# Y-Claw/Multilevel-GNN

Hardware: AMD Instinct MI355X
Metric: graphs/sec fwd+bwd, 3-level GNN on 10k-node d=128 synthetic; HBM GB/s %peak (higher is better)
Workload: dtype f32; 1 GPU; configs[1]: ER graphs N=10000 E=160000 x64 per GPU, d=128, 3 GENConv(softmax, res+, LayerNorm) + projection pooling G=25000 k=2 + DiffPool 146->37->10, fp32; step = CSR build (of the next batch, on a second stream) + fwd + bwd + grad all-reduce + Adam; graphs_per_gpu=64, global_batch=64, parallelism=dp1, world_size=1, allreduce_bytes=1429768

## Files before the change

multilevel-gnn_amd/csrc/densesage.hip:

```cpp
#include "common.h"
#include "mlgnn.h"
#include "tile_gemm.h"

namespace mlgnn {

constexpr int kDsMaxN = 160, kDsMaxC = 128, kDsMaxO = 64, kDsMaxNAdj = 48;
constexpr int kDsBlock = 1024, kDsWaves = kDsBlock / kWave;
constexpr int kDsSO = kDsMaxO + 1;
constexpr float kDsNormEps = 1e-12f;

struct DsArgs {
  const void* x; const void* adj; const void* w_rel; const void* w_root; const float* bias;
  const void* gy; const void* y; const float* rinv_in;
  void* y_out; float* rinv; void* gx; void* gadj; float* ws;
  int n; int C; int O; int adj_batched; int normalize; int ws_cols;
};

template <typename AB>
__device__ __forceinline__ void ds_degrees(const AB ab, int n, float* deg, float* raw) {
  const int lane = threadIdx.x & (kWave - 1), wave = threadIdx.x / kWave;
  for (int r = wave; r < n; r += kDsWaves) {
    float s = 0.f;
    for (int j = lane; j < n; j += kWave) s += ab[(size_t)r * n + j];
#pragma unroll
    for (int off = 32; off > 0; off >>= 1) s += __shfl_xor(s, off);
    if (lane == 0) {
      if (raw) raw[r] = s;
      deg[r] = fmaxf(s, 1.0f);
    }
  }
}

struct DsLds { int so, sx, np; };
__host__ __device__ inline DsLds ds_lds(int n, int C, int O) {
  DsLds l;
  l.np = (n + 15) & ~15;
  l.so = ((O + 15) & ~15) + 1;
  l.sx = C + 1 + (C & 1);
  return l;
}
inline size_t ds_fwd_lds_bytes(int n, int C, int O) {
  const DsLds l = ds_lds(n, C, O);
  return ((size_t)l.np * l.so + (size_t)l.np * l.sx + l.np) * 4;
}
inline size_t ds_bwd_lds_bytes(int n, int C, int O, bool adj_grad) {
  const DsLds l = ds_lds(n, C, O);
  size_t f = (size_t)2 * l.np * l.so + 2 * l.np;
  if (adj_grad) f += (size_t)l.np * l.so + (size_t)l.np * (l.np + 1);
  return f * 4;
}

template <typename T>
__global__ __launch_bounds__(kDsBlock) void dense_sage_fwd_kernel(const DsArgs p) {
  extern __shared__ __attribute__((aligned(16))) float ds_smem[];
  const int b = blockIdx.x, tid = threadIdx.x;
  const int lane = tid & (kWave - 1), wave = tid / kWave;
  const int n = p.n, C = p.C, O = p.O;
  const DsLds L = ds_lds(n, C, O);
  const int SO = L.so, SX = L.sx;
  float* Pm_ = ds_smem;
  float* Xm_ = Pm_ + (size_t)L.np * SO;
  float* deg = Xm_ + (size_t)L.np * SX;
#define P(r, c) Pm_[(r) * SO + (c)]
#define X(r, c) Xm_[(r) * SX + (c)]
  const StoredIn<T> xb{static_cast<const T*>(p.x) + (size_t)b * n * C};
  const StoredIn<T> ab{static_cast<const T*>(p.adj) + (p.adj_batched ? (size_t)b * n * n : 0)};
  const StoredIn<T> w_rel{static_cast<const T*>(p.w_rel)}, w_root{static_cast<const T*>(p.w_root)};
  const int NP = (n + 15) & ~15, OP = (O + 15) & ~15;
  const int Nt = NP / 16, Ot = OP / 16;
  const int l15 = lane & 15, lq = lane >> 4;

  ds_degrees(ab, n, deg, nullptr);
  for (int idx = tid; idx < NP * C; idx += kDsBlock) {
    const int r = idx / C, c = idx % C;
    X(r, c) = r < n ? xb[idx] : 0.f;
  }
  __syncthreads();
  for (int t = wave; t < Nt * Ot; t += kDsWaves) {
    const int i0 = (t / Ot) * 16, j0 = (t % Ot) * 16;
    const f32x4 acc = tile_gemm(C,
        [&](int i, int k) { return k < C ? X(i0 + i, k) : 0.f; },
        [&](int k, int j) { return (j0 + j < O && k < C) ? w_rel[(size_t)(j0 + j) * C + k] : 0.f; });
#pragma unroll
    for (int r = 0; r < 4; ++r) P(i0 + lq * 4 + r, j0 + l15) = acc[r];
  }
  __syncthreads();
  f32x4 keep[(kDsMaxN / 16) * (kDsMaxO / 16) / kDsWaves + 1];
  int nk = 0;
  for (int t = wave; t < Nt * Ot; t += kDsWaves, ++nk) {
    const int i0 = (t / Ot) * 16, j0 = (t % Ot) * 16;
    f32x4 acc = tile_gemm(n,
        [&](int i, int k) { return (i0 + i < n && k < n) ? ab[(size_t)(i0 + i) * n + k] : 0.f; },
        [&](int k, int j) { return k < n ? P(k, j0 + j) : 0.f; });
    const f32x4 root = tile_gemm(C,
        [&](int i, int k) { return k < C ? X(i0 + i, k) : 0.f; },
        [&](int k, int j) { return (j0 + j < O && k < C) ? w_root[(size_t)(j0 + j) * C + k] : 0.f; });
    const float bj = (p.bias && j0 + l15 < O) ? p.bias[j0 + l15] : 0.f;
#pragma unroll
    for (int r = 0; r < 4; ++r) {
      const int row = i0 + lq * 4 + r;
      acc[r] = acc[r] / deg[min(row, n - 1)] + root[r] + bj;
    }
    keep[nk] = acc;
  }
  __syncthreads();
  nk = 0;
  for (int t = wave; t < Nt * Ot; t += kDsWaves, ++nk) {
    const int i0 = (t / Ot) * 16, j0 = (t % Ot) * 16;
#pragma unroll
    for (int r = 0; r < 4; ++r) P(i0 + lq * 4 + r, j0 + l15) = keep[nk][r];
  }
  __syncthreads();
  for (int r = wave; r < n; r += kDsWaves) {
    const float v = lane < O ? P(r, lane) : 0.f;
    float ss = v * v;
#pragma unroll
    for (int off = 32; off > 0; off >>= 1) ss += __shfl_xor(ss, off);
    const float ri = p.normalize ? 1.0f / fmaxf(sqrtf(ss), kDsNormEps) : 1.0f;
    if (lane < O) stored_write<T>(p.y_out, ((size_t)b * n + r) * O + lane, v * ri);
    if (lane == 0) p.rinv[(size_t)b * n + r] = ri;
  }
}
#undef P
#undef X

template <typename T>
__global__ __launch_bounds__(kDsBlock) void dense_sage_bwd_kernel(const DsArgs p) {
  extern __shared__ __attribute__((aligned(16))) float ds_smem[];
  const int b = blockIdx.x, tid = threadIdx.x;
  const int lane = tid & (kWave - 1), wave = tid / kWave;
  const int n = p.n, C = p.C, O = p.O;
  const DsLds L = ds_lds(n, C, O);
  const int SO = L.so, SM = L.np + 1;
  float* G_ = ds_smem;
  float* GP_ = G_ + (size_t)L.np * SO;
  float* deg = GP_ + (size_t)L.np * SO;
  float* raw = deg + L.np;
  float* Pm_ = raw + L.np;
  float* M_ = Pm_ + (size_t)L.np * SO;
#define G(r, c) G_[(r) * SO + (c)]
#define GP(r, c) GP_[(r) * SO + (c)]
#define Pm(r, c) Pm_[(r) * SO + (c)]
#define M(r, c) M_[(r) * SM + (c)]
  const StoredIn<T> xb{static_cast<const T*>(p.x) + (size_t)b * n * C};
  const StoredIn<T> ab{static_cast<const T*>(p.adj) + (p.adj_batched ? (size_t)b * n * n : 0)};
  const StoredIn<T> w_rel{static_cast<const T*>(p.w_rel)}, w_root{static_cast<const T*>(p.w_root)};
  const StoredIn<T> gyb{static_cast<const T*>(p.gy) + (size_t)b * n * O};
  const StoredIn<T> yb{static_cast<const T*>(p.y) + (size_t)b * n * O};
  const int NP = (n + 15) & ~15, OP = (O + 15) & ~15, CP = (C + 15) & ~15;
  const int Nt = NP / 16, Ot = OP / 16, Ct = CP / 16;
  const int l15 = lane & 15, lq = lane >> 4;

  ds_degrees(ab, n, deg, raw);
  for (int r = wave; r < NP; r += kDsWaves) {
    float gv = 0.f, yv = 0.f;
    if (r < n && lane < O) { gv = gyb[(size_t)r * O + lane]; yv = yb[(size_t)r * O + lane]; }
    float dot = gv * yv;
#pragma unroll
    for (int off = 32; off > 0; off >>= 1) dot += __shfl_xor(dot, off);
    const float ri = r < n ? p.rinv_in[(size_t)b * n + r] : 0.f;
    const float g = p.normalize ? (gv - yv * dot) * ri : gv;
    if (lane < OP) G(r, lane) = (r < n && lane < O) ? g : 0.f;
  }
  __syncthreads();
  for (int t = wave; t < Nt * Ot; t += kDsWaves) {
    const int i0 = (t / Ot) * 16, j0 = (t % Ot) * 16;
    const f32x4 acc = tile_gemm(n,
        [&](int i, int k) { return (i0 + i < n && k < n) ? ab[(size_t)k * n + i0 + i] : 0.f; },
        [&](int k, int j) { return k < n ? G(k, j0 + j) / deg[k] : 0.f; });
#pragma unroll
    for (int r = 0; r < 4; ++r) GP(i0 + lq * 4 + r, j0 + l15) = acc[r];
  }
  __syncthreads();
  const size_t gx_off = (size_t)b * n * C;
  for (int t = wave; t < Nt * Ct; t += kDsWaves) {
    const int i0 = (t / Ct) * 16, c0 = (t % Ct) * 16;
    f32x4 acc = tile_gemm(O,
        [&](int i, int k) { return k < O ? GP(i0 + i, k) : 0.f; },
        [&](int k, int j) { return (k < O && c0 + j < C) ? w_rel[(size_t)k * C + c0 + j] : 0.f; });
    const f32x4 t2 = tile_gemm(O,
        [&](int i, int k) { return k < O ? G(i0 + i, k) : 0.f; },
        [&](int k, int j) { return (k < O && c0 + j < C) ? w_root[(size_t)k * C + c0 + j] : 0.f; });
#pragma unroll
    for (int r = 0; r < 4; ++r) {
      const int row = i0 + lq * 4 + r, col = c0 + l15;
      if (row < n && col < C) stored_write<T>(p.gx, gx_off + (size_t)row * C + col, acc[r] + t2[r]);
    }
  }
  float* wsb = p.ws + (size_t)b * p.ws_cols;
  for (int t = wave; t < 2 * Ot * Ct; t += kDsWaves) {
    const int which = t / (Ot * Ct), tt = t % (Ot * Ct);
    const int o0 = (tt / Ct) * 16, c0 = (tt % Ct) * 16;
    const float* src = which == 0 ? GP_ : G_;
    const f32x4 acc = tile_gemm(n,
        [&](int i, int k) { return k < n ? src[k * SO + o0 + i] : 0.f; },
        [&](int k, int j) { return (k < n && c0 + j < C) ? xb[(size_t)k * C + c0 + j] : 0.f; });
#pragma unroll
    for (int r = 0; r < 4; ++r) {
      const int o = o0 + lq * 4 + r, c = c0 + l15;
      if (o < O && c < C) wsb[(size_t)which * O * C + (size_t)o * C + c] = acc[r];
    }
  }
  for (int o = tid; o < O; o += kDsBlock) {
    float s = 0.f;
    for (int r = 0; r < n; ++r) s += G(r, o);
    wsb[(size_t)2 * O * C + o] = s;
  }
  if (p.gadj) {
    for (int t = wave; t < Nt * Ot; t += kDsWaves) {
      const int i0 = (t / Ot) * 16, j0 = (t % Ot) * 16;
      const f32x4 acc = tile_gemm(C,
          [&](int i, int k) { return (i0 + i < n && k < C) ? xb[(size_t)(i0 + i) * C + k] : 0.f; },
          [&](int k, int j) { return (j0 + j < O && k < C) ? w_rel[(size_t)(j0 + j) * C + k] : 0.f; });
#pragma unroll
      for (int r = 0; r < 4; ++r) Pm(i0 + lq * 4 + r, j0 + l15) = acc[r];
    }
    __syncthreads();
    for (int t = wave; t < Nt * Nt; t += kDsWaves) {
      const int i0 = (t / Nt) * 16, j0 = (t % Nt) * 16;
      const f32x4 acc = tile_gemm(O,
          [&](int i, int k) { return k < O ? G(i0 + i, k) : 0.f; },
          [&](int k, int j) { return k < O ? Pm(j0 + j, k) : 0.f; });
#pragma unroll
      for (int r = 0; r < 4; ++r) M(i0 + lq * 4 + r, j0 + l15) = acc[r];
    }
    __syncthreads();
    const size_t ga_off = (size_t)b * n * n;
    for (int r = wave; r < n; r += kDsWaves) {
      float c = lane < n ? ab[(size_t)r * n + lane] * M(r, lane) : 0.f;
#pragma unroll
      for (int off = 32; off > 0; off >>= 1) c += __shfl_xor(c, off);
      const float ci = raw[r] > 1.0f ? c / deg[r] : 0.f;
      if (lane < n) stored_write<T>(p.gadj, ga_off + (size_t)r * n + lane, (M(r, lane) - ci) / deg[r]);
    }
  }
}
#undef G
#undef GP
#undef Pm
#undef M

static bool ds_dims_ok(int64_t n, int64_t C, int64_t O) {
  return n >= 1 && n <= kDsMaxN && C >= 1 && C <= kDsMaxC && O >= 1 && O <= kDsMaxO;
}

}

using namespace mlgnn;

extern "C" int mlgnn_dense_sage_supported(int64_t n, int64_t C, int64_t O, int need_grad_adj) {
  return (ds_dims_ok(n, C, O) && (!need_grad_adj || n <= kDsMaxNAdj)) ? 1 : 0;
}

extern "C" int64_t mlgnn_dense_sage_bwd_workspace_floats(int64_t B, int64_t C, int64_t O) {
  if (B < 0 || C <= 0 || O <= 0) return MLGNN_E_SHAPE;
  return B * (2 * O * C + O);
}

extern "C" int mlgnn_dense_sage_fwd(const void* x, const void* adj, const void* w_rel, const void* w_root,
                                    const float* bias, void* y, float* rinv, int64_t B, int64_t n, int64_t C,
                                    int64_t O, int adj_batched, int normalize, int dtype, void* stream) {
  if (dtype != MLGNN_DTYPE_F32 && dtype != MLGNN_DTYPE_BF16) return MLGNN_E_DTYPE;
  if (B < 0 || !ds_dims_ok(n, C, O)) return MLGNN_E_SHAPE;
  if (B == 0) return 0;
  if (!x || !adj || !w_rel || !w_root || !y || !rinv) return MLGNN_E_NULL;
  DsArgs a = {};
  a.x = x; a.adj = adj; a.w_rel = w_rel; a.w_root = w_root;
  a.bias = bias; a.y_out = y; a.rinv = rinv;
  a.n = (int)n; a.C = (int)C; a.O = (int)O; a.adj_batched = adj_batched; a.normalize = normalize;
  const size_t lds = ds_fwd_lds_bytes((int)n, (int)C, (int)O);
  static size_t fwd_attr = 0;
  if (lds > fwd_attr) {
    const int most = (int)ds_fwd_lds_bytes(kDsMaxN, kDsMaxC, kDsMaxO);
    (void)hipFuncSetAttribute(reinterpret_cast<const void*>(&dense_sage_fwd_kernel<float>), hipFuncAttributeMaxDynamicSharedMemorySize, most);
    (void)hipFuncSetAttribute(reinterpret_cast<const void*>(&dense_sage_fwd_kernel<bf16_t>), hipFuncAttributeMaxDynamicSharedMemorySize, most);
    fwd_attr = (size_t)most;
  }
  if (dtype == MLGNN_DTYPE_BF16) hipLaunchKernelGGL(dense_sage_fwd_kernel<bf16_t>, dim3((unsigned)B), dim3(kDsBlock), lds, (hipStream_t)stream, a);
  else hipLaunchKernelGGL(dense_sage_fwd_kernel<float>, dim3((unsigned)B), dim3(kDsBlock), lds, (hipStream_t)stream, a);
  return (int)hipGetLastError();
}

extern "C" int mlgnn_dense_sage_bwd(const void* grad_y, const void* y, const float* rinv, const void* x,
                                    const void* adj, const void* w_rel, const void* w_root, void* grad_x,
                                    void* grad_adj, float* grad_w, float* workspace, int64_t workspace_floats,
                                    int64_t B, int64_t n, int64_t C, int64_t O, int adj_batched, int normalize,
                                    int dtype, void* stream) {
  if (dtype != MLGNN_DTYPE_F32 && dtype != MLGNN_DTYPE_BF16) return MLGNN_E_DTYPE;
  if (B < 0 || !ds_dims_ok(n, C, O)) return MLGNN_E_SHAPE;
  if (grad_adj && n > kDsMaxNAdj) return MLGNN_E_SHAPE;
  if (!grad_w) return MLGNN_E_NULL;
  const int cols = (int)(2 * O * C + O);
  hipStream_t s = (hipStream_t)stream;
  if (B == 0) return (int)hipMemsetAsync(grad_w, 0, (size_t)cols * 4, s);
  if (!grad_y || !y || !rinv || !x || !adj || !w_rel || !w_root || !grad_x || !workspace) return MLGNN_E_NULL;
  if (workspace_floats < B * cols) return MLGNN_E_WORKSPACE;
  DsArgs a = {};
  a.x = x; a.adj = adj; a.w_rel = w_rel; a.w_root = w_root;
  a.gy = grad_y; a.y = y; a.rinv_in = rinv;
  a.gx = grad_x; a.gadj = grad_adj; a.ws = workspace; a.ws_cols = cols;
  a.n = (int)n; a.C = (int)C; a.O = (int)O; a.adj_batched = adj_batched; a.normalize = normalize;
  const size_t lds = ds_bwd_lds_bytes((int)n, (int)C, (int)O, grad_adj != nullptr);
  static size_t bwd_attr = 0;
  if (lds > bwd_attr) {
    const size_t most = ds_bwd_lds_bytes(kDsMaxN, kDsMaxC, kDsMaxO, false) > ds_bwd_lds_bytes(kDsMaxNAdj, kDsMaxC, kDsMaxO, true)
                            ? ds_bwd_lds_bytes(kDsMaxN, kDsMaxC, kDsMaxO, false) : ds_bwd_lds_bytes(kDsMaxNAdj, kDsMaxC, kDsMaxO, true);
    (void)hipFuncSetAttribute(reinterpret_cast<const void*>(&dense_sage_bwd_kernel<float>), hipFuncAttributeMaxDynamicSharedMemorySize, (int)most);
    (void)hipFuncSetAttribute(reinterpret_cast<const void*>(&dense_sage_bwd_kernel<bf16_t>), hipFuncAttributeMaxDynamicSharedMemorySize, (int)most);
    bwd_attr = most;
  }
  if (dtype == MLGNN_DTYPE_BF16) hipLaunchKernelGGL(dense_sage_bwd_kernel<bf16_t>, dim3((unsigned)B), dim3(kDsBlock), lds, s, a);
  else hipLaunchKernelGGL(dense_sage_bwd_kernel<float>, dim3((unsigned)B), dim3(kDsBlock), lds, s, a);
  int err = (int)hipGetLastError();
  if (err) return err;
  launch_reduce_partials(workspace, grad_w, (int)B, cols, s);
  return (int)hipGetLastError();
}
```

multilevel-gnn_amd/csrc/tile_gemm.h:

```cpp
#pragma once
#include "common.h"

namespace mlgnn {

using f32x4 = __attribute__((ext_vector_type(4))) float;

constexpr int kTileUnroll = 8;

template <typename FA, typename FB>
__device__ __forceinline__ f32x4 tile_gemm(int kdim, FA a_at, FB b_at) {
  const int lane = threadIdx.x & (kWave - 1);
  const int l15 = lane & 15, lk = lane >> 4;
  f32x4 acc = {0.f, 0.f, 0.f, 0.f};
  for (int k0 = 0; k0 < kdim; k0 += 4 * kTileUnroll) {
    float a[kTileUnroll], b[kTileUnroll];
#pragma unroll
    for (int u = 0; u < kTileUnroll; ++u) {
      a[u] = a_at(l15, k0 + 4 * u + lk);
      b[u] = b_at(k0 + 4 * u + lk, l15);
    }
#pragma unroll
    for (int u = 0; u < kTileUnroll; ++u) acc = __builtin_amdgcn_mfma_f32_16x16x4f32(a[u], b[u], acc, 0, 0, 0);
  }
  return acc;
}

}
```

Before: 5504 graphs/s.

## Stage dense SAGE operands in LDS and interleave two MFMA tiles per wave

The DiffPool dense SAGE forward and backward kernels now copy x, the adjacency and both weight matrices into LDS through a multi-row staging helper, instead of having every MFMA tile reread them from global memory. The GEMMs run through a new LDS tile_gemm that computes two independent accumulators at once, and degree sums are taken from the staged adjacency. LDS regions are reused through explicit layout plans, and the row count per wave is a template parameter with a small-n variant. This cuts redundant global loads and exposes more MFMA ILP, at the cost of more LDS and register pressure and more complex buffer aliasing.

```diff
diff --git a/multilevel-gnn_amd/csrc/densesage.hip b/multilevel-gnn_amd/csrc/densesage.hip
--- a/multilevel-gnn_amd/csrc/densesage.hip
+++ b/multilevel-gnn_amd/csrc/densesage.hip
@@ -16,128 +16,234 @@
   int n; int C; int O; int adj_batched; int normalize; int ws_cols;
 };
 
-template <typename AB>
-__device__ __forceinline__ void ds_degrees(const AB ab, int n, float* deg, float* raw) {
+constexpr int kDsRows = kDsMaxN / kDsWaves, kDsRowsSmall = 3;
+template <int ROWS>
+__device__ __forceinline__ void ds_degrees(const float* adj, int sa, int n, float* deg, float* raw, float (&sum)[ROWS]) {
   const int lane = threadIdx.x & (kWave - 1), wave = threadIdx.x / kWave;
-  for (int r = wave; r < n; r += kDsWaves) {
-    float s = 0.f;
-    for (int j = lane; j < n; j += kWave) s += ab[(size_t)r * n + j];
-#pragma unroll
-    for (int off = 32; off > 0; off >>= 1) s += __shfl_xor(s, off);
-    if (lane == 0) {
-      if (raw) raw[r] = s;
-      deg[r] = fmaxf(s, 1.0f);
-    }
-  }
-}
-
-struct DsLds { int so, sx, np; };
-__host__ __device__ inline DsLds ds_lds(int n, int C, int O) {
-  DsLds l;
-  l.np = (n + 15) & ~15;
-  l.so = ((O + 15) & ~15) + 1;
-  l.sx = C + 1 + (C & 1);
+#pragma unroll
+  for (int u = 0; u < ROWS; ++u) sum[u] = 0.f;
+  for (int j = lane; j < n; j += kWave) {
+#pragma unroll
+    for (int u = 0; u < ROWS; ++u) sum[u] += adj[min(wave + u * kDsWaves, n - 1) * sa + j];
+  }
+#pragma unroll
+  for (int off = 32; off > 0; off >>= 1) {
+#pragma unroll
+    for (int u = 0; u < ROWS; ++u) sum[u] += __shfl_xor(sum[u], off);
+  }
+#pragma unroll
+  for (int u = 0; u < ROWS; ++u) {
+    const int r = wave + u * kDsWaves;
+    if (lane == 0 && r < n) {
+      if (raw) raw[r] = sum[u];
+      deg[r] = fmaxf(sum[u], 1.0f);
+    }
+  }
+}
+template <int ROWS>
+__device__ __forceinline__ void ds_degrees(const float* adj, int sa, int n, float* deg) {
+  float sum[ROWS];
+  ds_degrees<ROWS>(adj, sa, n, deg, nullptr, sum);
+}
+
+constexpr int kDsLdsFloats = 40000;
+constexpr int kDsMaxKeep = 4;
+
+struct DsFwdPlan {
+  int np, op, cp, so, sx, sa;
+  int deg, x, wrel, wroot, p, adj, total;
+};
+__host__ __device__ inline DsFwdPlan ds_fwd_plan(int n, int C, int O) {
+  DsFwdPlan l;
+  l.np = (n + 15) & ~15; l.op = (O + 15) & ~15; l.cp = (C + 15) & ~15;
+  l.so = l.op + 1; l.sx = l.cp + 1; l.sa = l.np + 1;
+  l.deg = 0;
+  const int base = l.np;
+  l.x = base; l.wrel = l.x + l.np * l.sx; l.wroot = l.wrel + l.op * l.sx;
+  const int end1 = l.wroot + l.op * l.sx;
+  l.p = base; l.adj = l.p + l.np * l.so;
+  const int end2 = l.adj + l.np * l.sa;
+  l.total = end1 > end2 ? end1 : end2;
   return l;
 }
-inline size_t ds_fwd_lds_bytes(int n, int C, int O) {
-  const DsLds l = ds_lds(n, C, O);
-  return ((size_t)l.np * l.so + (size_t)l.np * l.sx + l.np) * 4;
-}
-inline size_t ds_bwd_lds_bytes(int n, int C, int O, bool adj_grad) {
-  const DsLds l = ds_lds(n, C, O);
-  size_t f = (size_t)2 * l.np * l.so + 2 * l.np;
-  if (adj_grad) f += (size_t)l.np * l.so + (size_t)l.np * (l.np + 1);
-  return f * 4;
-}
-
-template <typename T>
+inline size_t ds_fwd_lds_bytes(int n, int C, int O) { return (size_t)ds_fwd_plan(n, C, O).total * 4; }
+
+struct DsBwdPlan {
+  int np, op, cp, so, sa, sc, ch, chp, sxc;
+  int deg, raw, g, gp, adj, wrel, wroot, x, pm, m, total;
+};
+__host__ __device__ inline DsBwdPlan ds_bwd_plan(int n, int C, int O, bool adj_grad) {
+  DsBwdPlan l;
+  l.np = (n + 15) & ~15; l.op = (O + 15) & ~15; l.cp = (C + 15) & ~15;
+  l.so = l.op + 1; l.sa = l.np + 1; l.sc = l.cp + 1;
+  l.deg = 0; l.raw = l.np;
+  l.g = 2 * l.np; l.gp = l.g + l.np * l.so;
+  l.adj = l.gp;
+  int end = l.adj + l.np * l.sa;
+  l.wrel = l.gp + l.np * l.so; l.wroot = l.wrel + l.op * l.sc;
+  const int wend = l.wroot + l.op * l.sc;
+  end = wend > end ? wend : end;
+  l.x = adj_grad ? wend : l.wrel;
+  l.ch = C; l.chp = l.cp;
+  if (!adj_grad && l.x + l.np * (l.cp + 1) > kDsLdsFloats) { l.ch = 64; l.chp = 64; }
+  l.sxc = l.chp + 1;
+  const int xend = l.x + l.np * l.sxc;
+  end = xend > end ? xend : end;
+  l.pm = xend; l.m = l.pm + l.np * l.so;
+  if (adj_grad) end = l.m + l.np * l.sa;
+  l.total = end;
+  return l;
+}
+inline size_t ds_bwd_lds_bytes(int n, int C, int O, bool adj_grad) { return (size_t)ds_bwd_plan(n, C, O, adj_grad).total * 4; }
+
+constexpr int kDsStageCols = 2;
+template <int ROWS, typename SRC>
+__device__ __forceinline__ void ds_stage(float* img, int stride, const SRC src, int rows, int cols, int src_stride,
+                                         int rows_p, int cols_p) {
+  const int lane = threadIdx.x & (kWave - 1), wave = threadIdx.x / kWave;
+  for (int r0 = wave; r0 < rows_p; r0 += kDsWaves * ROWS) {
+    for (int c0 = lane; c0 < cols_p; c0 += kWave * kDsStageCols) {
+      float v[kDsStageCols][ROWS];
+#pragma unroll
+      for (int h = 0; h < kDsStageCols; ++h) {
+#pragma unroll
+        for (int u = 0; u < ROWS; ++u) {
+          const int r = r0 + u * kDsWaves, c = c0 + h * kWave;
+          const bool ok = r < rows && c < cols;
+          const float got = src[ok ? (size_t)r * src_stride + c : 0];
+          v[h][u] = ok ? got : 0.f;
+        }
+      }
+#pragma unroll
+      for (int h = 0; h < kDsStageCols; ++h) {
+#pragma unroll
+        for (int u = 0; u < ROWS; ++u) {
+          const int r = r0 + u * kDsWaves, c = c0 + h * kWave;
+          if (r < rows_p && c < cols_p) img[r * stride + c] = v[h][u];
+        }
+      }
+    }
+  }
+}
+
+template <typename T, int ROWS>
 __global__ __launch_bounds__(kDsBlock) void dense_sage_fwd_kernel(const DsArgs p) {
   extern __shared__ __attribute__((aligned(16))) float ds_smem[];
   const int b = blockIdx.x, tid = threadIdx.x;
   const int lane = tid & (kWave - 1), wave = tid / kWave;
   const int n = p.n, C = p.C, O = p.O;
-  const DsLds L = ds_lds(n, C, O);
-  const int SO = L.so, SX = L.sx;
-  float* Pm_ = ds_smem;
-  float* Xm_ = Pm_ + (size_t)L.np * SO;
-  float* deg = Xm_ + (size_t)L.np * SX;
+  const DsFwdPlan L = ds_fwd_plan(n, C, O);
+  const int SO = L.so, SX = L.sx, SA = L.sa;
+  float* deg = ds_smem + L.deg;
+  float* Xm_ = ds_smem + L.x;
+  float* Wr_ = ds_smem + L.wrel;
+  float* Wo_ = ds_smem + L.wroot;
+  float* Pm_ = ds_smem + L.p;
+  float* Am_ = ds_smem + L.adj;
 #define P(r, c) Pm_[(r) * SO + (c)]
-#define X(r, c) Xm_[(r) * SX + (c)]
   const StoredIn<T> xb{static_cast<const T*>(p.x) + (size_t)b * n * C};
   const StoredIn<T> ab{static_cast<const T*>(p.adj) + (p.adj_batched ? (size_t)b * n * n : 0)};
   const StoredIn<T> w_rel{static_cast<const T*>(p.w_rel)}, w_root{static_cast<const T*>(p.w_root)};
-  const int NP = (n + 15) & ~15, OP = (O + 15) & ~15;
-  const int Nt = NP / 16, Ot = OP / 16;
+  const int NP = L.np, OP = L.op, CP = L.cp;
+  const int Nt = NP / 16, Ot = OP / 16, T_ = Nt * Ot;
   const int l15 = lane & 15, lq = lane >> 4;
 
-  ds_degrees(ab, n, deg, nullptr);
-  for (int idx = tid; idx < NP * C; idx += kDsBlock) {
-    const int r = idx / C, c = idx % C;
-    X(r, c) = r < n ? xb[idx] : 0.f;
-  }
-  __syncthreads();
-  for (int t = wave; t < Nt * Ot; t += kDsWaves) {
-    const int i0 = (t / Ot) * 16, j0 = (t % Ot) * 16;
-    const f32x4 acc = tile_gemm(C,
-        [&](int i, int k) { return k < C ? X(i0 + i, k) : 0.f; },
-        [&](int k, int j) { return (j0 + j < O && k < C) ? w_rel[(size_t)(j0 + j) * C + k] : 0.f; });
-#pragma unroll
-    for (int r = 0; r < 4; ++r) P(i0 + lq * 4 + r, j0 + l15) = acc[r];
-  }
-  __syncthreads();
-  f32x4 keep[(kDsMaxN / 16) * (kDsMaxO / 16) / kDsWaves + 1];
-  int nk = 0;
-  for (int t = wave; t < Nt * Ot; t += kDsWaves, ++nk) {
-    const int i0 = (t / Ot) * 16, j0 = (t % Ot) * 16;
-    f32x4 acc = tile_gemm(n,
-        [&](int i, int k) { return (i0 + i < n && k < n) ? ab[(size_t)(i0 + i) * n + k] : 0.f; },
-        [&](int k, int j) { return k < n ? P(k, j0 + j) : 0.f; });
-    const f32x4 root = tile_gemm(C,
-        [&](int i, int k) { return k < C ? X(i0 + i, k) : 0.f; },
-        [&](int k, int j) { return (j0 + j < O && k < C) ? w_root[(size_t)(j0 + j) * C + k] : 0.f; });
-    const float bj = (p.bias && j0 + l15 < O) ? p.bias[j0 + l15] : 0.f;
-#pragma unroll
-    for (int r = 0; r < 4; ++r) {
-      const int row = i0 + lq * 4 + r;
-      acc[r] = acc[r] / deg[min(row, n - 1)] + root[r] + bj;
-    }
-    keep[nk] = acc;
-  }
-  __syncthreads();
-  nk = 0;
-  for (int t = wave; t < Nt * Ot; t += kDsWaves, ++nk) {
-    const int i0 = (t / Ot) * 16, j0 = (t % Ot) * 16;
-#pragma unroll
-    for (int r = 0; r < 4; ++r) P(i0 + lq * 4 + r, j0 + l15) = keep[nk][r];
-  }
-  __syncthreads();
-  for (int r = wave; r < n; r += kDsWaves) {
-    const float v = lane < O ? P(r, lane) : 0.f;
-    float ss = v * v;
-#pragma unroll
-    for (int off = 32; off > 0; off >>= 1) ss += __shfl_xor(ss, off);
-    const float ri = p.normalize ? 1.0f / fmaxf(sqrtf(ss), kDsNormEps) : 1.0f;
-    if (lane < O) stored_write<T>(p.y_out, ((size_t)b * n + r) * O + lane, v * ri);
-    if (lane == 0) p.rinv[(size_t)b * n + r] = ri;
+  ds_stage<ROWS>(Xm_, SX, xb, n, C, C, NP, CP);
+  ds_stage<ROWS>(Wr_, SX, w_rel, O, C, C, OP, CP);
+  ds_stage<ROWS>(Wo_, SX, w_root, O, C, C, OP, CP);
+  __syncthreads();
+  f32x4 keepP[kDsMaxKeep], keepR[kDsMaxKeep];
+#pragma unroll
+  for (int q = 0; q < kDsMaxKeep; ++q) {
+    const int t = wave + q * kDsWaves;
+    if (t < T_) {
+      const int i0 = (t / Ot) * 16, j0 = (t % Ot) * 16;
+      const LdsOperand xa{Xm_ + (i0 + l15) * SX + lq, 1};
+      tile_gemm_lds2(CP, xa, LdsOperand{Wr_ + (j0 + l15) * SX + lq, 1}, xa, LdsOperand{Wo_ + (j0 + l15) * SX + lq, 1},
+                     keepP[q], keepR[q]);
+    }
+  }
+  __syncthreads();
+  ds_stage<ROWS>(Am_, SA, ab, n, n, n, NP, NP);
+#pragma unroll
+  for (int q = 0; q < kDsMaxKeep; ++q) {
+    const int t = wave + q * kDsWaves;
+    if (t < T_) {
+      const int i0 = (t / Ot) * 16, j0 = (t % Ot) * 16;
+#pragma unroll
+      for (int r = 0; r < 4; ++r) P(i0 + lq * 4 + r, j0 + l15) = keepP[q][r];
+    }
+  }
+  __syncthreads();
+#pragma unroll
+  for (int q = 0; q < kDsMaxKeep; q += 2) {
+    const int t = wave + q * kDsWaves;
+    if (t < T_) {
+      const bool two = t + kDsWaves < T_;
+      const int t1 = two ? t + kDsWaves : t;
+      const int i0 = (t / Ot) * 16, j0 = (t % Ot) * 16, i1 = (t1 / Ot) * 16, j1 = (t1 % Ot) * 16;
+      f32x4 acc0, acc1;
+      tile_gemm_lds2(NP, LdsOperand{Am_ + (i0 + l15) * SA + lq, 1}, LdsOperand{Pm_ + lq * SO + j0 + l15, SO},
+                     LdsOperand{Am_ + (i1 + l15) * SA + lq, 1}, LdsOperand{Pm_ + lq * SO + j1 + l15, SO}, acc0, acc1);
+      keepP[q] = acc0;
+      if (two) keepP[q + 1] = acc1;
+    }
+  }
+  ds_degrees<ROWS>(Am_, SA, n, deg);
+  __syncthreads();
+#pragma unroll
+  for (int q = 0; q < kDsMaxKeep; ++q) {
+    const int t = wave + q * kDsWaves;
+    if (t < T_) {
+      const int i0 = (t / Ot) * 16, j0 = (t % Ot) * 16;
+      const float bj = (p.bias && j0 + l15 < O) ? p.bias[j0 + l15] : 0.f;
+#pragma unroll
+      for (int r = 0; r < 4; ++r) {
+        const int row = i0 + lq * 4 + r;
+        P(row, j0 + l15) = keepP[q][r] / deg[min(row, n - 1)] + keepR[q][r] + bj;
+      }
+    }
+  }
+  __syncthreads();
+  float v[ROWS], ss[ROWS];
+#pragma unroll
+  for (int u = 0; u < ROWS; ++u) {
+    v[u] = lane < O ? P(min(wave + u * kDsWaves, n - 1), lane) : 0.f;
+    ss[u] = v[u] * v[u];
+  }
+#pragma unroll
+  for (int off = 32; off > 0; off >>= 1) {
+#pragma unroll
+    for (int u = 0; u < ROWS; ++u) ss[u] += __shfl_xor(ss[u], off);
+  }
+#pragma unroll
+  for (int u = 0; u < ROWS; ++u) {
+    const int r = wave + u * kDsWaves;
+    const float ri = p.normalize ? 1.0f / fmaxf(sqrtf(ss[u]), kDsNormEps) : 1.0f;
+    if (r < n && lane < O) stored_write<T>(p.y_out, ((size_t)b * n + r) * O + lane, v[u] * ri);
+    if (r < n && lane == 0) p.rinv[(size_t)b * n + r] = ri;
   }
 }
 #undef P
-#undef X
-
-template <typename T>
+
+template <typename T, int ROWS>
 __global__ __launch_bounds__(kDsBlock) void dense_sage_bwd_kernel(const DsArgs p) {
   extern __shared__ __attribute__((aligned(16))) float ds_smem[];
   const int b = blockIdx.x, tid = threadIdx.x;
   const int lane = tid & (kWave - 1), wave = tid / kWave;
   const int n = p.n, C = p.C, O = p.O;
-  const DsLds L = ds_lds(n, C, O);
-  const int SO = L.so, SM = L.np + 1;
-  float* G_ = ds_smem;
-  float* GP_ = G_ + (size_t)L.np * SO;
-  float* deg = GP_ + (size_t)L.np * SO;
-  float* raw = deg + L.np;
-  float* Pm_ = raw + L.np;
-  float* M_ = Pm_ + (size_t)L.np * SO;
+  const DsBwdPlan L = ds_bwd_plan(n, C, O, p.gadj != nullptr);
+  const int SO = L.so, SA = L.sa, SC = L.sc, SM = L.sa;
+  float* deg = ds_smem + L.deg;
+  float* raw = ds_smem + L.raw;
+  float* G_ = ds_smem + L.g;
+  float* GP_ = ds_smem + L.gp;
+  float* Am_ = ds_smem + L.adj;
+  float* Wr_ = ds_smem + L.wrel;
+  float* Wo_ = ds_smem + L.wroot;
+  float* Xm_ = ds_smem + L.x;
+  float* Pm_ = ds_smem + L.pm;
+  float* M_ = ds_smem + L.m;
 #define G(r, c) G_[(r) * SO + (c)]
 #define GP(r, c) GP_[(r) * SO + (c)]
 #define Pm(r, c) Pm_[(r) * SO + (c)]
@@ -147,40 +253,76 @@
   const StoredIn<T> w_rel{static_cast<const T*>(p.w_rel)}, w_root{static_cast<const T*>(p.w_root)};
   const StoredIn<T> gyb{static_cast<const T*>(p.gy) + (size_t)b * n * O};
   const StoredIn<T> yb{static_cast<const T*>(p.y) + (size_t)b * n * O};
-  const int NP = (n + 15) & ~15, OP = (O + 15) & ~15, CP = (C + 15) & ~15;
+  const int NP = L.np, OP = L.op, CP = L.cp;
   const int Nt = NP / 16, Ot = OP / 16, Ct = CP / 16;
   const int l15 = lane & 15, lq = lane >> 4;
 
-  ds_degrees(ab, n, deg, raw);
-  for (int r = wave; r < NP; r += kDsWaves) {
-    float gv = 0.f, yv = 0.f;
-    if (r < n && lane < O) { gv = gyb[(size_t)r * O + lane]; yv = yb[(size_t)r * O + lane]; }
-    float dot = gv * yv;
+  constexpr int kRows = ROWS;
+  float gk[kRows], yk[kRows], rk[kRows];
+#pragma unroll
+  for (int u = 0; u < kRows; ++u) {
+    const int r = wave + u * kDsWaves;
+    const bool ok = r < n && lane < O;
+    const size_t at = ok ? (size_t)r * O + lane : 0;
+    const float gv = gyb[at], yv = yb[at];
+    rk[u] = p.rinv_in[(size_t)b * n + min(r, n - 1)];
+    gk[u] = ok ? gv : 0.f;
+    yk[u] = ok ? yv : 0.f;
+  }
+  ds_stage<ROWS>(Am_, SA, ab, n, n, n, NP, NP);
+#pragma unroll
+  for (int u = 0; u < kRows; ++u) {
+    float dot = gk[u] * yk[u];
 #pragma unroll
     for (int off = 32; off > 0; off >>= 1) dot += __shfl_xor(dot, off);
-    const float ri = r < n ? p.rinv_in[(size_t)b * n + r] : 0.f;
-    const float g = p.normalize ? (gv - yv * dot) * ri : gv;
-    if (lane < OP) G(r, lane) = (r < n && lane < O) ? g : 0.f;
-  }
-  __syncthreads();
-  for (int t = wave; t < Nt * Ot; t += kDsWaves) {
-    const int i0 = (t / Ot) * 16, j0 = (t % Ot) * 16;
-    const f32x4 acc = tile_gemm(n,
-        [&](int i, int k) { return (i0 + i < n && k < n) ? ab[(size_t)k * n + i0 + i] : 0.f; },
-        [&](int k, int j) { return k < n ? G(k, j0 + j) / deg[k] : 0.f; });
-#pragma unroll
-    for (int r = 0; r < 4; ++r) GP(i0 + lq * 4 + r, j0 + l15) = acc[r];
-  }
+    if (p.normalize) gk[u] = (gk[u] - yk[u] * dot) * rk[u];
+  }
+  __syncthreads();
+  float rowsum[kRows];
+  ds_degrees(Am_, SA, n, deg, raw, rowsum);
+#pragma unroll
+  for (int u = 0; u < kRows; ++u) {
+    const int r = wave + u * kDsWaves;
+    if (r < NP && lane < OP) G(r, lane) = (r < n && lane < O) ? gk[u] / fmaxf(rowsum[u], 1.0f) : 0.f;
+  }
+  __syncthreads();
+  f32x4 keep[kDsMaxKeep];
+  const int T_ = Nt * Ot;
+#pragma unroll
+  for (int q = 0; q < kDsMaxKeep; q += 2) {
+    const int t = wave + q * kDsWaves;
+    if (t < T_) {
+      const int t1 = t + kDsWaves < T_ ? t + kDsWaves : t;
+      const int i0 = (t / Ot) * 16, j0 = (t % Ot) * 16, i1 = (t1 / Ot) * 16, j1 = (t1 % Ot) * 16;
+      tile_gemm_lds2(NP, LdsOperand{Am_ + lq * SA + i0 + l15, SA}, LdsOperand{G_ + lq * SO + j0 + l15, SO},
+                     LdsOperand{Am_ + lq * SA + i1 + l15, SA}, LdsOperand{G_ + lq * SO + j1 + l15, SO},
+                     keep[q], keep[q + 1]);
+    }
+  }
+  __syncthreads();
+#pragma unroll
+  for (int q = 0; q < kDsMaxKeep; ++q) {
+    const int t = wave + q * kDsWaves;
+    if (t < T_) {
+      const int i0 = (t / Ot) * 16, j0 = (t % Ot) * 16;
+#pragma unroll
+      for (int r = 0; r < 4; ++r) GP(i0 + lq * 4 + r, j0 + l15) = keep[q][r];
+    }
+  }
+#pragma unroll
+  for (int u = 0; u < kRows; ++u) {
+    const int r = wave + u * kDsWaves;
+    if (r < NP && lane < OP) G(r, lane) = (r < n && lane < O) ? gk[u] : 0.f;
+  }
+  ds_stage<ROWS>(Wr_, SC, w_rel, O, C, C, OP, CP);
+  ds_stage<ROWS>(Wo_, SC, w_root, O, C, C, OP, CP);
   __syncthreads();
   const size_t gx_off = (size_t)b * n * C;
   for (int t = wave; t < Nt * Ct; t += kDsWaves) {
     const int i0 = (t / Ct) * 16, c0 = (t % Ct) * 16;
-    f32x4 acc = tile_gemm(O,
-        [&](int i, int k) { return k < O ? GP(i0 + i, k) : 0.f; },
-        [&](int k, int j) { return (k < O && c0 + j < C) ? w_rel[(size_t)k * C + c0 + j] : 0.f; });
-    const f32x4 t2 = tile_gemm(O,
-        [&](int i, int k) { return k < O ? G(i0 + i, k) : 0.f; },
-        [&](int k, int j) { return (k < O && c0 + j < C) ? w_root[(size_t)k * C + c0 + j] : 0.f; });
+    f32x4 acc, t2;
+    tile_gemm_lds2(OP, LdsOperand{GP_ + (i0 + l15) * SO + lq, 1}, LdsOperand{Wr_ + lq * SC + c0 + l15, SC},
+                   LdsOperand{G_ + (i0 + l15) * SO + lq, 1}, LdsOperand{Wo_ + lq * SC + c0 + l15, SC}, acc, t2);
 #pragma unroll
     for (int r = 0; r < 4; ++r) {
       const int row = i0 + lq * 4 + r, col = c0 + l15;
@@ -188,41 +330,73 @@
     }
   }
   float* wsb = p.ws + (size_t)b * p.ws_cols;
-  for (int t = wave; t < 2 * Ot * Ct; t += kDsWaves) {
-    const int which = t / (Ot * Ct), tt = t % (Ot * Ct);
-    const int o0 = (tt / Ct) * 16, c0 = (tt % Ct) * 16;
-    const float* src = which == 0 ? GP_ : G_;
-    const f32x4 acc = tile_gemm(n,
-        [&](int i, int k) { return k < n ? src[k * SO + o0 + i] : 0.f; },
-        [&](int k, int j) { return (k < n && c0 + j < C) ? xb[(size_t)k * C + c0 + j] : 0.f; });
-#pragma unroll
-    for (int r = 0; r < 4; ++r) {
-      const int o = o0 + lq * 4 + r, c = c0 + l15;
-      if (o < O && c < C) wsb[(size_t)which * O * C + (size_t)o * C + c] = acc[r];
-    }
-  }
   for (int o = tid; o < O; o += kDsBlock) {
     float s = 0.f;
-    for (int r = 0; r < n; ++r) s += G(r, o);
+    for (int r0 = 0; r0 < NP; r0 += 16) {
+      float gv[16];
+#pragma unroll
+      for (int i = 0; i < 16; ++i) gv[i] = G(r0 + i, o);
+#pragma unroll
+      for (int i = 0; i < 16; ++i) s += gv[i];
+    }
     wsb[(size_t)2 * O * C + o] = s;
   }
+  for (int cc = 0; cc < C; cc += L.ch) {
+    if (!p.gadj || cc > 0) __syncthreads();
+    const int cw = min(L.ch, C - cc), cwp = (cw + 15) & ~15, Cc = cwp / 16;
+    ds_stage<ROWS>(Xm_, L.sxc, StoredIn<T>{xb.p + cc}, n, cw, C, NP, cwp);
+    __syncthreads();
+    const int Tw = 2 * Ot * Cc;
+    for (int t0 = wave; t0 < Tw; t0 += 3 * kDsWaves) {
+      int which[3], o0[3], c0[3];
+      LdsOperand ta[3], tb[3];
+#pragma unroll
+      for (int h = 0; h < 3; ++h) {
+        const int t = t0 + h * kDsWaves < Tw ? t0 + h * kDsWaves : t0, tt = t % (Ot * Cc);
+        which[h] = t / (Ot * Cc); o0[h] = (tt / Cc) * 16; c0[h] = (tt % Cc) * 16;
+        ta[h] = LdsOperand{(which[h] == 0 ? GP_ : G_) + lq * SO + o0[h] + l15, SO};
+        tb[h] = LdsOperand{Xm_ + lq * L.sxc + c0[h] + l15, L.sxc};
+      }
+      f32x4 acc[3];
+      tile_gemm_lds<3>(NP, ta, tb, acc);
+#pragma unroll
+      for (int h = 0; h < 3; ++h) {
+        if (h == 0 || t0 + h * kDsWaves < Tw) {
+#pragma unroll
+          for (int r = 0; r < 4; ++r) {
+            const int o = o0[h] + lq * 4 + r, c = cc + c0[h] + l15;
+            if (o < O && c < C) wsb[(size_t)which[h] * O * C + (size_t)o * C + c] = acc[h][r];
+          }
+        }
+      }
+    }
+  }
   if (p.gadj) {
-    for (int t = wave; t < Nt * Ot; t += kDsWaves) {
-      const int i0 = (t / Ot) * 16, j0 = (t % Ot) * 16;
-      const f32x4 acc = tile_gemm(C,
-          [&](int i, int k) { return (i0 + i < n && k < C) ? xb[(size_t)(i0 + i) * C + k] : 0.f; },
-          [&](int k, int j) { return (j0 + j < O && k < C) ? w_rel[(size_t)(j0 + j) * C + k] : 0.f; });
-#pragma unroll
-      for (int r = 0; r < 4; ++r) Pm(i0 + lq * 4 + r, j0 + l15) = acc[r];
+    const int SX = L.sxc;
+    for (int t = wave; t < Nt * Ot; t += 2 * kDsWaves) {
+      const int t1 = t + kDsWaves < Nt * Ot ? t + kDsWaves : t;
+      const int i0 = (t / Ot) * 16, j0 = (t % Ot) * 16, i1 = (t1 / Ot) * 16, j1 = (t1 % Ot) * 16;
+      f32x4 acc0, acc1;
+      tile_gemm_lds2(CP, LdsOperand{Xm_ + (i0 + l15) * SX + lq, 1}, LdsOperand{Wr_ + (j0 + l15) * SC + lq, 1},
+                     LdsOperand{Xm_ + (i1 + l15) * SX + lq, 1}, LdsOperand{Wr_ + (j1 + l15) * SC + lq, 1}, acc0, acc1);
+#pragma unroll
+      for (int r = 0; r < 4; ++r) {
+        Pm(i0 + lq * 4 + r, j0 + l15) = acc0[r];
+        if (t1 != t) Pm(i1 + lq * 4 + r, j1 + l15) = acc1[r];
+      }
     }
     __syncthreads();
-    for (int t = wave; t < Nt * Nt; t += kDsWaves) {
-      const int i0 = (t / Nt) * 16, j0 = (t % Nt) * 16;
-      const f32x4 acc = tile_gemm(O,
-          [&](int i, int k) { return k < O ? G(i0 + i, k) : 0.f; },
-          [&](int k, int j) { return k < O ? Pm(j0 + j, k) : 0.f; });
-#pragma unroll
-      for (int r = 0; r < 4; ++r) M(i0 + lq * 4 + r, j0 + l15) = acc[r];
+    for (int t = wave; t < Nt * Nt; t += 2 * kDsWaves) {
+      const int t1 = t + kDsWaves < Nt * Nt ? t + kDsWaves : t;
+      const int i0 = (t / Nt) * 16, j0 = (t % Nt) * 16, i1 = (t1 / Nt) * 16, j1 = (t1 % Nt) * 16;
+      f32x4 acc0, acc1;
+      tile_gemm_lds2(OP, LdsOperand{G_ + (i0 + l15) * SO + lq, 1}, LdsOperand{Pm_ + (j0 + l15) * SO + lq, 1},
+                     LdsOperand{G_ + (i1 + l15) * SO + lq, 1}, LdsOperand{Pm_ + (j1 + l15) * SO + lq, 1}, acc0, acc1);
+#pragma unroll
+      for (int r = 0; r < 4; ++r) {
+        M(i0 + lq * 4 + r, j0 + l15) = acc0[r];
+        if (t1 != t) M(i1 + lq * 4 + r, j1 + l15) = acc1[r];
+      }
     }
     __syncthreads();
     const size_t ga_off = (size_t)b * n * n;
@@ -269,15 +443,22 @@
   a.bias = bias; a.y_out = y; a.rinv = rinv;
   a.n = (int)n; a.C = (int)C; a.O = (int)O; a.adj_batched = adj_batched; a.normalize = normalize;
   const size_t lds = ds_fwd_lds_bytes((int)n, (int)C, (int)O);
-  static size_t fwd_attr = 0;
-  if (lds > fwd_attr) {
+  const bool small = n <= 16 * kDsRowsSmall;
+  const void* fn = dtype == MLGNN_DTYPE_BF16
+      ? (small ? reinterpret_cast<const void*>(&dense_sage_fwd_kernel<bf16_t, kDsRowsSmall>) : reinterpret_cast<const void*>(&dense_sage_fwd_kernel<bf16_t, kDsRows>))
+      : (small ? reinterpret_cast<const void*>(&dense_sage_fwd_kernel<float, kDsRowsSmall>) : reinterpret_cast<const void*>(&dense_sage_fwd_kernel<float, kDsRows>));
+  static bool fwd_attr = false;
+  if (!fwd_attr) {
     const int most = (int)ds_fwd_lds_bytes(kDsMaxN, kDsMaxC, kDsMaxO);
-    (void)hipFuncSetAttribute(reinterpret_cast<const void*>(&dense_sage_fwd_kernel<float>), hipFuncAttributeMaxDynamicSharedMemorySize, most);
-    (void)hipFuncSetAttribute(reinterpret_cast<const void*>(&dense_sage_fwd_kernel<bf16_t>), hipFuncAttributeMaxDynamicSharedMemorySize, most);
-    fwd_attr = (size_t)most;
-  }
-  if (dtype == MLGNN_DTYPE_BF16) hipLaunchKernelGGL(dense_sage_fwd_kernel<bf16_t>, dim3((unsigned)B), dim3(kDsBlock), lds, (hipStream_t)stream, a);
-  else hipLaunchKernelGGL(dense_sage_fwd_kernel<float>, dim3((unsigned)B), dim3(kDsBlock), lds, (hipStream_t)stream, a);
+    (void)hipFuncSetAttribute(reinterpret_cast<const void*>(&dense_sage_fwd_kernel<float, kDsRows>), hipFuncAttributeMaxDynamicSharedMemorySize, most);
+    (void)hipFuncSetAttribute(reinterpret_cast<const void*>(&dense_sage_fwd_kernel<bf16_t, kDsRows>), hipFuncAttributeMaxDynamicSharedMemorySize, most);
+    (void)hipFuncSetAttribute(reinterpret_cast<const void*>(&dense_sage_fwd_kernel<float, kDsRowsSmall>), hipFuncAttributeMaxDynamicSharedMemorySize, most);
+    (void)hipFuncSetAttribute(reinterpret_cast<const void*>(&dense_sage_fwd_kernel<bf16_t, kDsRowsSmall>), hipFuncAttributeMaxDynamicSharedMemorySize, most);
+    fwd_attr = true;
+  }
+  void* params[] = {&a};
+  int err = (int)hipLaunchKernel(fn, dim3((unsigned)B), dim3(kDsBlock), params, lds, (hipStream_t)stream);
+  if (err) return err;
   return (int)hipGetLastError();
 }
 
@@ -301,17 +482,22 @@
   a.gx = grad_x; a.gadj = grad_adj; a.ws = workspace; a.ws_cols = cols;
   a.n = (int)n; a.C = (int)C; a.O = (int)O; a.adj_batched = adj_batched; a.normalize = normalize;
   const size_t lds = ds_bwd_lds_bytes((int)n, (int)C, (int)O, grad_adj != nullptr);
-  static size_t bwd_attr = 0;
-  if (lds > bwd_attr) {
+  const bool small = n <= 16 * kDsRowsSmall;
+  const void* fn = dtype == MLGNN_DTYPE_BF16
+      ? (small ? reinterpret_cast<const void*>(&dense_sage_bwd_kernel<bf16_t, kDsRowsSmall>) : reinterpret_cast<const void*>(&dense_sage_bwd_kernel<bf16_t, kDsRows>))
+      : (small ? reinterpret_cast<const void*>(&dense_sage_bwd_kernel<float, kDsRowsSmall>) : reinterpret_cast<const void*>(&dense_sage_bwd_kernel<float, kDsRows>));
+  static bool bwd_attr = false;
+  if (!bwd_attr) {
     const size_t most = ds_bwd_lds_bytes(kDsMaxN, kDsMaxC, kDsMaxO, false) > ds_bwd_lds_bytes(kDsMaxNAdj, kDsMaxC, kDsMaxO, true)
                             ? ds_bwd_lds_bytes(kDsMaxN, kDsMaxC, kDsMaxO, false) : ds_bwd_lds_bytes(kDsMaxNAdj, kDsMaxC, kDsMaxO, true);
-    (void)hipFuncSetAttribute(reinterpret_cast<const void*>(&dense_sage_bwd_kernel<float>), hipFuncAttributeMaxDynamicSharedMemorySize, (int)most);
-    (void)hipFuncSetAttribute(reinterpret_cast<const void*>(&dense_sage_bwd_kernel<bf16_t>), hipFuncAttributeMaxDynamicSharedMemorySize, (int)most);
-    bwd_attr = most;
-  }
-  if (dtype == MLGNN_DTYPE_BF16) hipLaunchKernelGGL(dense_sage_bwd_kernel<bf16_t>, dim3((unsigned)B), dim3(kDsBlock), lds, s, a);
-  else hipLaunchKernelGGL(dense_sage_bwd_kernel<float>, dim3((unsigned)B), dim3(kDsBlock), lds, s, a);
-  int err = (int)hipGetLastError();
+    (void)hipFuncSetAttribute(reinterpret_cast<const void*>(&dense_sage_bwd_kernel<float, kDsRows>), hipFuncAttributeMaxDynamicSharedMemorySize, (int)most);
+    (void)hipFuncSetAttribute(reinterpret_cast<const void*>(&dense_sage_bwd_kernel<bf16_t, kDsRows>), hipFuncAttributeMaxDynamicSharedMemorySize, (int)most);
+    (void)hipFuncSetAttribute(reinterpret_cast<const void*>(&dense_sage_bwd_kernel<float, kDsRowsSmall>), hipFuncAttributeMaxDynamicSharedMemorySize, (int)most);
+    (void)hipFuncSetAttribute(reinterpret_cast<const void*>(&dense_sage_bwd_kernel<bf16_t, kDsRowsSmall>), hipFuncAttributeMaxDynamicSharedMemorySize, (int)most);
+    bwd_attr = true;
+  }
+  void* params[] = {&a};
+  int err = (int)hipLaunchKernel(fn, dim3((unsigned)B), dim3(kDsBlock), params, lds, s);
   if (err) return err;
   launch_reduce_partials(workspace, grad_w, (int)B, cols, s);
   return (int)hipGetLastError();
diff --git a/multilevel-gnn_amd/csrc/tile_gemm.h b/multilevel-gnn_amd/csrc/tile_gemm.h
--- a/multilevel-gnn_amd/csrc/tile_gemm.h
+++ b/multilevel-gnn_amd/csrc/tile_gemm.h
@@ -25,4 +25,41 @@
   return acc;
 }
 
+struct LdsOperand {
+  const float* p;
+  int sk;
+};
+
+template <int NC>
+__device__ __forceinline__ void tile_gemm_lds(int kp, const LdsOperand (&a)[NC], const LdsOperand (&b)[NC], f32x4 (&acc)[NC]) {
+  constexpr int U = 4;
+#pragma unroll
+  for (int c = 0; c < NC; ++c) acc[c] = f32x4{0.f, 0.f, 0.f, 0.f};
+  for (int k0 = 0; k0 < kp; k0 += 4 * U) {
+    float ca[NC][U], cb[NC][U];
+#pragma unroll
+    for (int c = 0; c < NC; ++c) {
+#pragma unroll
+      for (int u = 0; u < U; ++u) {
+        ca[c][u] = a[c].p[(k0 + 4 * u) * a[c].sk];
+        cb[c][u] = b[c].p[(k0 + 4 * u) * b[c].sk];
+      }
+    }
+#pragma unroll
+    for (int u = 0; u < U; ++u) {
+#pragma unroll
+      for (int c = 0; c < NC; ++c) acc[c] = __builtin_amdgcn_mfma_f32_16x16x4f32(ca[c][u], cb[c][u], acc[c], 0, 0, 0);
+    }
+  }
 }
+
+__device__ __forceinline__ void tile_gemm_lds2(int kp, LdsOperand a0, LdsOperand b0, LdsOperand a1, LdsOperand b1,
+                                               f32x4& acc0, f32x4& acc1) {
+  const LdsOperand a[2] = {a0, a1}, b[2] = {b0, b1};
+  f32x4 acc[2];
+  tile_gemm_lds<2>(kp, a, b, acc);
+  acc0 = acc[0];
+  acc1 = acc[1];
+}
+
+}
```

Measured after the change: 5580 graphs/s, median of 6. 1.01x the previous value.
